# ChaissonLab/danbing-tk

Hardware: AMD Instinct MI355X
Metric: paired reads/sec aligned to RPGG (k=21) (higher is better)
Workload: dtype u64; 1 GPU; release-scale synthetic RPGG (80000 loci, 143352206 index keys, 31153328 TR k-mers) replicated per GPU; 10000000 x 150bp PE reads per GPU per step, 2% of pairs from loci; -k 21 -kf 4 1 -cth 45 -ka; RCCL all-reduce of counts at the end; lanes=1, reads_per_gpu=10000000, read_len=150, k=21, cth=45

## Files before the change

### danbing-tk_amd/csrc/dbtk_probe2.h

```cpp
#ifndef DBTK_PROBE2_H_
#define DBTK_PROBE2_H_

namespace dbtk {

#ifndef DBTK_P2_RCH
#define DBTK_P2_RCH 40
#endif
constexpr int P2_RCH = DBTK_P2_RCH;
constexpr int P2_ROW = 9;
constexpr int P2_CACHE = 128;
struct P2FuseArgs {
    uint64_t* counts; uint64_t* nmapread; uint64_t* kmc;
    uint32_t* gen_list; uint32_t* ngen; uint32_t* walk_dst;
    const uint8_t* qc;
    const ClsSlot* cls; uint64_t cls_mask; uint32_t cls_shift;
    uint64_t* pstats;
    uint64_t* ctr;
    uint32_t ctr_rep;
    dbtk_params_t P;
};
template <int NPL>
struct __attribute__((aligned(16))) Probe2SmemT {
    uint32_t pk[2][20];
    uint16_t vd[2][40];
    uint32_t rb[64 * NPL];
    union {
        uint4 stg[P2_RCH][P2_ROW];
        uint32_t res[2][2][32 * NPL];
    };
    uint4 cache[P2_CACHE];
    uint8_t tok[P2_CACHE];
    uint32_t gbuf[64];
    uint32_t fc[12];
    P2FuseArgs fa;
};
constexpr uint32_t P2_HWIN = 2048;
constexpr uint32_t P2_REP_DONE = 24, P2_REP_CLS = 25, P2_REP_INC = 26, P2_REP_SHARED = 27;
#ifndef DBTK_P2_SHARED_MAX
#define DBTK_P2_SHARED_MAX 48
#endif
constexpr uint32_t P2_SHARED_MAX = DBTK_P2_SHARED_MAX;
static_assert(P2_HWIN / 2 * 4 <= sizeof(uint4) * P2_RCH * P2_ROW, "the counter window fits where the buckets were");

template <int NPL, int WN>
DBTK_HD void sliding_min(const uint32_t (&f)[NPL + WN - 1], uint32_t (&out)[NPL]) {
    static_assert(WN >= NPL, "the windows of one lane share at least one element");
    uint32_t c = f[NPL - 1];
#pragma unroll
    for (int t = NPL; t < WN; ++t) c = f[t] < c ? f[t] : c;
    uint32_t suf[NPL];
    suf[NPL - 1] = 0xFFFFFFFFu;
#pragma unroll
    for (int j = NPL - 2; j >= 0; --j) suf[j] = f[j] < suf[j + 1] ? f[j] : suf[j + 1];
    uint32_t pre = 0xFFFFFFFFu;
#pragma unroll
    for (int j = 0; j < NPL; ++j) {
        uint32_t v = suf[j] < c ? suf[j] : c;
        out[j] = pre < v ? pre : v;
        if (j + 1 < NPL) pre = f[WN + j] < pre ? f[WN + j] : pre;
    }
}

#ifdef DBTK_STAMPS
#define P2_DIAG_MASK(a) (((a).P.diag & 512) ? 127u : 0xFFFFFFFFu)
#else
#define P2_DIAG_MASK(a) 0xFFFFFFFFu
#endif
typedef uint32_t p2_v4u __attribute__((vector_size(16)));
DBTK_HD void p2_fetch_runs(const uint32_t* rb, const MzBucket* mz, uint32_t nruns, uint32_t r0, uint32_t fq8, uint32_t part, uint32_t bmask,
                           p2_v4u (&q)[P2_RCH / 8]) {
#pragma unroll
    for (int u = 0; u < P2_RCH / 8; ++u) {
        const uint32_t run = r0 + 8 * u + fq8;
        const uint32_t b = rb[run < nruns ? run : 0u] & bmask;
        q[u] = reinterpret_cast<const p2_v4u*>(mz + (run < nruns ? (size_t)b : (size_t)0))[part];
    }
}

template <int NPL> struct P2Rv { uint64_t v[NPL]; };
enum { P2C_QC, P2C_KF, P2C_THR, P2C_FEAS, P2C_ASGN, P2C_CLS, P2C_INC, P2C_NHASH1, P2C_DONE, P2C_VV, P2C_SHARED, P2C_HF };
template <int NPL, class SM, class X>
DBTK_HD_NOINLINE void p2_resolve_gone(X& x, SM& sm_, P2Rv<NPL> rv, uint32_t nk, uint32_t gmask, uint32_t rsh, uint32_t k) {
    SM& sm = DBTK_LDS_REF(SM, sm_);
    const int lane = x.lane();
    const uint32_t hl = (uint32_t)lane & 31u, half = (uint32_t)lane >> 5, p0 = hl * NPL, cth = sm.fa.P.cthreshold;
    const bool mygone = ((gmask >> half) & 1u) != 0;
    uint32_t mc = 0;
#pragma unroll
    for (int j = 0; j < NPL; ++j) mc += (p0 + j < nk && (uint32_t)rv.v[j] == NOHIT) ? 1u : 0u;
    uint32_t ex = x.wave_excl_scan(mc);
    const uint32_t ex32 = x.bcast(ex, 32);
    if (half) ex -= ex32;
    uint32_t upto = 0;
    if (mygone && nk >= cth) {
        const uint32_t target = nk - cth + 1;
#pragma unroll
        for (int j = 0; j < NPL; ++j)
            if (p0 + j < nk && (uint32_t)rv.v[j] == NOHIT) { ++ex; if (ex == target) upto = p0 + j + 1; }
    }
    if (!mygone) upto = nk;
    upto = x.half_max(upto);
    const uint32_t looked = x.bcast(upto, 0) + x.bcast(upto, 32);
    uint32_t nvv = 0;
    if (gmask != 3u) {
        bool sh[NPL];
        bool any = false;
#pragma unroll
        for (int j = 0; j < NPL; ++j) {
            sh[j] = !mygone && p0 + j < nk && (uint32_t)rv.v[j] != NOHIT && ((uint32_t)rv.v[j] & 1u);
            any |= sh[j];
        }
        if (x.ballot(any)) {
            const uint64_t kmask = (1ull << (2 * k)) - 1;
            const uint64_t W = window_fw_clean(sm.pk[half], rsh + p0, 32), RW = revcomp2(W, 32);
            uint64_t km[NPL];
            uint32_t mine = 0, dup = 0;
#pragma unroll
            for (int j = 0; j < NPL; ++j) {
                const uint64_t fw = (W >> (2 * (32 - k - j))) & kmask, rc = (RW >> (2 * j)) & kmask;
                km[j] = fw < rc ? fw : rc;
                mine += sh[j] ? 1u : 0u;
            }
#pragma unroll
            for (int j = 0; j < NPL; ++j) {
                uint64_t mj = x.ballot(sh[j]);
                while (mj) {
                    const int src = (int)__builtin_ctzll(mj);
                    mj &= mj - 1;
                    const uint64_t ke = ((uint64_t)x.bcast((uint32_t)(km[j] >> 32), src) << 32) | x.bcast((uint32_t)km[j], src);
#pragma unroll
                    for (int j2 = j; j2 < NPL; ++j2)
                        if (sh[j2] && km[j2] == ke && (j2 > j || lane > src)) dup |= 1u << j2;
                }
            }
            nvv = x.wave_sum(mine) - x.wave_sum((uint32_t)__builtin_popcount(dup));
        }
    }
    if (lane == 0) {
        sm.fc[P2C_NHASH1] += looked;
        sm.fc[P2C_KF] += (gmask & 1u) + (gmask >> 1);
        if (gmask != 3u) { sm.fc[P2C_HF] += 1; sm.fc[P2C_VV] += nvv; }
    }
}
template <int NPL, class SM, class X>
DBTK_HD_NOINLINE void p2_resolve_usual(X& x, SM& sm_, P2Rv<NPL> rv, uint32_t nk, uint32_t v0, uint32_t nks, uint32_t t) {
    SM& sm = DBTK_LDS_REF(SM, sm_);
    const int lane = x.lane();
    const uint32_t hl = (uint32_t)lane & 31u, half = (uint32_t)lane >> 5, p0 = hl * NPL;
    const P2FuseArgs& fa = sm.fa;
    auto tally = [&](int w, uint32_t v) { if (lane == 0) sm.fc[w] += v; };
    tally(P2C_DONE, 1);
    tally(P2C_NHASH1, nks);
    const uint32_t dst = v0 >> 1;
#if defined(DBTK_STAMPS) || defined(DBTK_LF_DIAG)
    if (fa.P.diag & 64) return;
#endif
    if (fa.P.qc && fa.qc && !fa.qc[dst]) { tally(P2C_QC, 2); return; }
    if (fa.P.threading) {
        tally(P2C_THR, 2);
        if (fa.P.threading == DBTK_THREADING_V13 && lane == 0) fa.walk_dst[t] = dst;
        return;
    }
    tally(P2C_THR, 2); tally(P2C_FEAS, 2);
    if (fa.P.extract) return;
    tally(P2C_CLS, nks);
    bool kn[NPL], tr[NPL];
    uint32_t anyk = 0, anyt = 0;
#pragma unroll
    for (int j = 0; j < NPL; ++j) {
        const uint32_t ax = (uint32_t)(rv.v[j] >> 32);
        kn[j] = p0 + j < nk && (uint32_t)rv.v[j] != NOHIT && ax != CLS_NONE;
        tr[j] = kn[j] && ax != CLS_FLANK;
        anyk |= kn[j] && !tr[j] ? 1u : 0u; anyt |= tr[j] ? 1u : 0u;
    }
    const uint64_t bt = x.ballot(anyt != 0), bf = x.ballot(anyk != 0);
    const bool t0 = (uint32_t)bt != 0, t1 = (bt >> 32) != 0, f0 = (uint32_t)bf != 0, f1 = (bf >> 32) != 0;
    bool rm = true;
    uint32_t span = 0;
    if ((t0 && f0) || (t1 && f1)) assign_halves<NPL>(x, kn, tr, p0, nk, fa.P, rm, span);
    else { const bool tmate = half ? t1 : t0; rm = !tmate; span = tmate ? nk : 0u; }
    const uint32_t rm0 = x.bcast(rm ? 1u : 0u, 0), rm1 = x.bcast(rm ? 1u : 0u, 32);
    if (rm0 && rm1) return;
    tally(P2C_ASGN, 2 - rm0 - rm1);
#if defined(DBTK_STAMPS) || defined(DBTK_LF_DIAG)
    if (fa.P.diag & 128) return;
#endif
    uint32_t mn = 0xFFFFFFFFu, mx = 0;
#pragma unroll
    for (int j = 0; j < NPL; ++j) {
        const uint32_t ax = (uint32_t)(rv.v[j] >> 32);
        if (tr[j] && !rm) { mn = ax < mn ? ax : mn; mx = ax > mx ? ax : mx; }
    }
    const uint32_t hmn2 = ~x.half_max(~mn), hmx2 = x.half_max(mx);
    const uint32_t mnA = x.bcast(hmn2, 0), mnB = x.bcast(hmn2, 32), mxA = x.bcast(hmx2, 0), mxB = x.bcast(hmx2, 32);
    const uint32_t base = mnA < mnB ? mnA : mnB, top = mxA > mxB ? mxA : mxB;
    const uint32_t win = top >= base ? (top - base + 1 < P2_HWIN ? top - base + 1 : P2_HWIN) : 0u;
    uint32_t* hist = reinterpret_cast<uint32_t*>(sm.stg);
    for (uint32_t w = (uint32_t)lane; w < (win + 1) / 2; w += 64) hist[w] = 0;
    x.sync();
    uint32_t ninc = 0;
#pragma unroll
    for (int j = 0; j < NPL; ++j) {
        const bool hit = tr[j] && !rm;
        if (hit) {
            const uint32_t ax = (uint32_t)(rv.v[j] >> 32), o = ax - base;
            if (o < win) x.lds_add(&hist[o >> 1], 1u << (16 * (o & 1)));
            else x.atomic_add(&fa.counts[ax], 1ull);
        }
        ninc += (uint32_t)__builtin_popcountll(x.ballot(hit));
    }
    tally(P2C_INC, ninc);
    x.sync();
    const uint32_t span0 = x.bcast(span, 0), span1 = x.bcast(span, 32);
#if defined(DBTK_STAMPS) || defined(DBTK_LF_DIAG)
    if (!(fa.P.diag & 16))
#endif
    if (lane == 0) {
        x.atomic_add(&fa.nmapread[dst], (uint64_t)(2 - rm0 - rm1));
        x.atomic_add(&fa.kmc[dst], (uint64_t)span0 + span1);
    }
#if defined(DBTK_STAMPS) || defined(DBTK_LF_DIAG)
    if (!(fa.P.diag & 4))
#endif
    for (uint32_t i = (uint32_t)lane; i < win; i += 64) {
        const uint32_t v = (hist[i >> 1] >> (16 * (i & 1))) & 0xFFFFu;
// ... 32 lines not shown
    uint32_t dup = 0;
#pragma unroll
    for (int j = 0; j < NPL; ++j) {
        uint64_t mj = x.ballot(sh[j]);
        while (mj) {
            const int src = (int)__builtin_ctzll(mj);
            mj &= mj - 1;
            const uint64_t ke = ((uint64_t)x.bcast((uint32_t)(km[j] >> 32), src) << 32) | x.bcast((uint32_t)km[j], src);
#pragma unroll
            for (int j2 = j; j2 < NPL; ++j2)
                if (sh[j2] && km[j2] == ke && (j2 > j || lane > src)) dup |= 1u << j2;
        }
    }
    const uint32_t nvv = nshared - x.wave_sum((uint32_t)__builtin_popcount(dup));
    if (lane == 0) { sm.fc[P2C_VV] += nvv; sm.fc[P2C_SHARED] += 1; }
    p2_resolve_usual<NPL>(x, sm, rv, nk, 2u * L, nks, t);
    return true;
}

template <int NPL, int WN, bool SEL, bool FUSE, class X>
DBTK_HD void body_probe2(X& x, const BatchArgs& a) {
    typedef Probe2SmemT<NPL> SM;
    SM& sm = *x.template smem<SM>();
    const int lane = x.lane();
    const uint32_t hl = (uint32_t)lane & 31u, half = (uint32_t)lane >> 5;
    const DevTables& T = a.T;
    const uint32_t k = T.ksize, m = T.mz_m;
    const uint32_t ns = *a.nsurv;
    const uint32_t tend = ns - a.t0 < a.tcap ? ns : a.t0 + a.tcap;
    const uint32_t npc = ns > a.t0 ? tend - a.t0 : 0;
    const uint32_t npr = SEL ? *a.nsel : npc;
    if (SEL && a.pstats && x.bid() == 0 && lane == 0 && npr) x.atomic_add(&a.pstats[6], (uint64_t)npr);
    const uint32_t per = (npr + x.nblocks() - 1) / x.nblocks();
    const uint64_t lo64 = (uint64_t)x.bid() * per;
    const uint32_t first = lo64 < npr ? (uint32_t)lo64 : npr, hi = lo64 + per < npr ? (uint32_t)(lo64 + per) : npr;
    const uint32_t lmax = 32u * NPL + m - 1;
    const uint64_t kmask = (1ull << (2 * k)) - 1;
    const uint32_t mmask = (uint32_t)((1ull << (2 * m)) - 1);
    const uint32_t p0 = hl * NPL;
    if (FUSE && lane < 12) sm.fc[lane] = 0;
    if (FUSE && lane == 0) {
        sm.fa.counts = a.counts; sm.fa.nmapread = a.nmapread; sm.fa.kmc = a.kmc; sm.fa.gen_list = a.gen_list; sm.fa.ngen = a.ngen;
        sm.fa.walk_dst = a.walk_dst; sm.fa.qc = a.T.qc; sm.fa.pstats = a.pstats; sm.fa.P = a.P;
        sm.fa.ctr = counters_of(x, a); sm.fa.ctr_rep = a.ctr_rep ? 1u : 0u;
        sm.fa.cls = a.T.cls; sm.fa.cls_mask = a.T.cls_mask; sm.fa.cls_shift = a.T.cls_shift;
    }
    const P2FuseArgs& fa = sm.fa;
    uint32_t ngb = 0;
    auto flush_gen = [&]() {
        x.sync();
        uint32_t base = 0;
        if (lane == 0) base = x.atomic_add(fa.ngen, ngb);
        base = x.bcast(base, 0);
        if ((uint32_t)lane < ngb) fa.gen_list[base + lane] = sm.gbuf[lane];
        x.sync();
        ngb = 0;
    };
    for (uint32_t e = (uint32_t)lane; e < (uint32_t)P2_CACHE; e += 64) sm.cache[e] = uint4{0xFFFFFFFFu, 0x3FFFFFFFu, 0u, 0u};
    auto place_of = [&](uint32_t i) -> uint32_t {
        const uint32_t ic = i < hi ? i : (first < hi ? first : 0u);
        return SEL ? (npr ? a.sel[ic] : 0u) : ic;
    };
    uint32_t rw0 = 0, rw1 = 0;
    uint64_t o0C = 0, o1C = 0;
    uint64_t o0B = 0, o1B = 0;
    uint32_t pairA = 0;
    uint32_t plN = 0;
    auto fetch_bytes = [&](uint64_t o0, uint64_t o1) {
        uint32_t len = (uint32_t)(o1 - o0);
        if (len > lmax) len = lmax;
        const uint64_t a0 = o0 & ~3ull;
        const uint32_t nw = ((uint32_t)(o0 - a0) + len + 3) >> 2;
        rw0 = *reinterpret_cast<const uint32_t*>(a.seq + (2 * hl < nw ? a0 + 8ull * hl : 0ull));
        rw1 = *reinterpret_cast<const uint32_t*>(a.seq + (2 * hl + 1 < nw ? a0 + 8ull * hl + 4 : 0ull));
    };
    auto fetch_offsets = [&](uint32_t pair) {
        const uint64_t r = 2 * (uint64_t)pair + half;
        o0B = a.off[r]; o1B = a.off[r + 1];
    };
    if (first < hi) {
        fetch_offsets(x.uni(a.surv[a.t0 + place_of(first)]));
        o0C = o0B; o1C = o1B;
        fetch_bytes(o0C, o1C);
        if (first + 1 < hi) fetch_offsets(x.uni(a.surv[a.t0 + place_of(first + 1)]));
        pairA = a.surv[a.t0 + place_of(first + 2)];
        plN = place_of(first + 3);
    }
    DBTK_STAMP_DECL
    for (uint32_t i = first; i < hi; ++i) {
        DBTK_STAMP(43);
        const uint64_t o0 = o0C, o1 = o1C;
        uint32_t len = (uint32_t)(o1 - o0);
        if (len > lmax) { *a.errflag = DBTK_ERR_READ_TOO_LONG; len = lmax; }
        const uint64_t a0 = o0 & ~3ull;
        const uint32_t rsh = (uint32_t)(o0 - a0);
        const uint32_t d0 = rw0, d1 = rw1;
        const uint32_t place_v = place_of(i);
        {
            const bool hasB = i + 1 < hi, hasA = i + 2 < hi;
            o0C = hasB ? o0B : 0ull; o1C = hasB ? o1B : 0ull;
            fetch_bytes(o0C, o1C);
            fetch_offsets(hasA ? x.uni(pairA) : x.uni(pairA) * 0u);
            pairA = a.surv[a.t0 + plN];
            plN = place_of(i + 4);
        }
        x.sync();
        uint32_t bad = 0;
        {
            const uint32_t c0 = pack4_b2(d0, &bad), c1 = pack4_b2(d1, &bad);
            reinterpret_cast<uint16_t*>(sm.pk[half])[hl ^ 1u] = (uint16_t)(((c0 >> 8) & 0xFF00u) | ((c1 >> 16) & 0xFFu));
        }
        const uint32_t nk = len >= k ? len - k + 1 : 0, nmm = len >= m ? len - m + 1 : 0;
        const bool clean = x.ballot(bad != 0 && 8 * hl < rsh + len) == 0;
        uint64_t rv[NPL];
        if (clean) {
            x.sync();
            const uint64_t W = window_fw_clean(sm.pk[half], rsh + p0, 32);
            const uint64_t RW = revcomp2(W, 32);
            uint32_t f[NPL + WN - 1];
#pragma unroll
            for (int j = 0; j < NPL; ++j) {
                const uint32_t fwm = (uint32_t)(W >> (2 * (32 - m - j))) & mmask, rcm = (uint32_t)(RW >> (2 * j)) & mmask;
                f[j] = p0 + j < nmm ? mmer_hash2(fwm, rcm) : 0xFFFFFFFFu;
            }
#pragma unroll
            for (int t = NPL; t < NPL + WN - 1; ++t) f[t] = x.shfl_down1(f[t - NPL]);
            uint64_t km[NPL];
            bool act[NPL];
#pragma unroll
            for (int j = 0; j < NPL; ++j) {
                const uint64_t fw = (W >> (2 * (32 - k - j))) & kmask, rc = (RW >> (2 * j)) & kmask;
                km[j] = fw < rc ? fw : rc;
                act[j] = p0 + j < nk;
                rv[j] = (uint64_t)NOHIT;
            }
            DBTK_STAMP(40);
            uint32_t mz[NPL], bk[NPL];
            sliding_min<NPL, WN>(f, mz);
            uint32_t cnt = 0;
            bool st[NPL];
#pragma unroll
            for (int j = 0; j < NPL; ++j) bk[j] = act[j] ? mz_bucket(mz[j] >> 4, (uint32_t)T.mz_mask) : 0xFFFFFFFFu;
            uint32_t prev = x.shfl_up1(bk[NPL - 1]);
            if (hl == 0) prev = 0xFFFFFFFEu;
#pragma unroll
            for (int j = 0; j < NPL; ++j) {
                st[j] = act[j] && bk[j] != prev;
                cnt += st[j] ? 1u : 0u;
                prev = bk[j];
            }
            uint32_t r = x.wave_excl_scan(cnt);
            const uint32_t nruns = x.bcast(r + cnt, 63);
            uint32_t rid[NPL];
#pragma unroll
            for (int j = 0; j < NPL; ++j) {
                if (st[j]) { sm.rb[r] = bk[j]; ++r; }
                rid[j] = r - 1;
            }
            x.sync();
            DBTK_STAMP(16);
            const uint32_t fq8 = (uint32_t)lane >> 3, part = (uint32_t)lane & 7u;
            p2_v4u q[P2_RCH / 8];
            p2_fetch_runs(sm.rb, T.mz, nruns, 0u, fq8, part, P2_DIAG_MASK(a), q);
            bool pend[NPL];
#pragma unroll
            for (int j = 0; j < NPL; ++j) pend[j] = false;
            for (uint32_t r0 = 0; r0 < nruns; r0 += P2_RCH) {
                x.sync();
#pragma unroll
                for (int u = 0; u < P2_RCH / 8; ++u) *reinterpret_cast<p2_v4u*>(&sm.stg[8 * u + fq8][part]) = q[u];
                if (r0 + P2_RCH < nruns)
                    p2_fetch_runs(sm.rb, T.mz, nruns, r0 + P2_RCH, fq8, part, P2_DIAG_MASK(a), q);
                x.sync();
#pragma unroll
                for (int j = 0; j < NPL; ++j) {
                    const uint32_t row = rid[j] - r0;
                    const bool mine = act[j] && row < (uint32_t)P2_RCH;
                    if (mine) {
                        const uint4* rp = sm.stg[row];
                        int hit = -1;
                        uint32_t w7 = 0;
#pragma unroll
                        for (int g = 0; g < 4; ++g) {
                            const uint4 kk = rp[g];
                            const uint64_t k0 = ((uint64_t)kk.y << 32) | kk.x, k1 = ((uint64_t)kk.w << 32) | kk.z;
                            if (k0 == km[j]) hit = 2 * g;
                            if ((g == 3 ? (k1 & ~MZ_TURNED) : k1) == km[j]) hit = 2 * g + 1;
                            if (g == 3) w7 = kk.w;
                        }
                        const uint32_t* pl = reinterpret_cast<const uint32_t*>(rp + 4) + 2 * (hit >= 0 ? hit : 0);
                        const uint64_t pv = (uint64_t)pl[0] | ((uint64_t)pl[1] << 32);
                        if (hit >= 0) rv[j] = pv;
                        else pend[j] = (w7 >> 31) != 0;
                    }
                }
            }
            DBTK_STAMP(18);
            bool anyp = false;
#pragma unroll
            for (int j = 0; j < NPL; ++j) anyp |= pend[j];
#ifdef DBTK_STAMPS
            if (a.P.diag & 256) anyp = false;
#endif
            if (x.ballot(anyp)) {
                uint32_t oh[NPL], oi[NPL];
                bool glob[NPL];
                anyp = false;
#pragma unroll
                for (int j = 0; j < NPL; ++j) {
                    oh[j] = ovf_hash(km[j]);
                    oi[j] = oh[j] & (uint32_t)T.ovf_mask;
                    glob[j] = false;
                    if (pend[j]) {
                        const uint4 c = sm.cache[(oh[j] >> 20) & (P2_CACHE - 1)];
                        if (c.x == (uint32_t)km[j] && c.y == (uint32_t)(km[j] >> 32)) { rv[j] = ((uint64_t)c.w << 32) | c.z; pend[j] = false; }
                        else glob[j] = true;
                    }
                    anyp |= pend[j];
                }
                if (x.ballot(anyp)) {
                    uint4 q2[NPL];
                    do {
#pragma unroll
                        for (int j = 0; j < NPL; ++j) q2[j] = reinterpret_cast<const uint4*>(T.ovf)[pend[j] ? oi[j] : 0u];
                        anyp = false;
#pragma unroll
                        for (int j = 0; j < NPL; ++j) {
                            if (!pend[j]) continue;
                            const uint64_t key = ((uint64_t)q2[j].y << 32) | q2[j].x;
                            if (key == km[j]) { rv[j] = ((uint64_t)q2[j].w << 32) | q2[j].z; pend[j] = false; }
                            else if (key == MZ_EMPTY) pend[j] = false;
                            else oi[j] = (oi[j] + 1) & (uint32_t)T.ovf_mask;
                            anyp |= pend[j];
                        }
                    } while (x.ballot(anyp));
#pragma unroll
                    for (int j = 0; j < NPL; ++j) if (glob[j]) sm.tok[(oh[j] >> 20) & (P2_CACHE - 1)] = (uint8_t)lane;
                    x.sync();
#pragma unroll
                    for (int j = 0; j < NPL; ++j) {
                        const uint32_t ce = (oh[j] >> 20) & (P2_CACHE - 1);
                        if (glob[j] && sm.tok[ce] == (uint8_t)lane)
                            sm.cache[ce] = uint4{(uint32_t)km[j], (uint32_t)(km[j] >> 32), (uint32_t)rv[j], (uint32_t)(rv[j] >> 32)};
                    }
                    x.sync();
                }
            }
            DBTK_STAMP(41);
        } else {
            uint32_t vb = 0;
#pragma unroll
            for (int e = 0; e < 8; ++e) {
                const uint32_t sidx = 8 * hl + e, by = ((e < 4 ? d0 : d1) >> (8 * (e & 3))) & 0xFFu;
                const bool ok = sidx >= rsh && sidx < rsh + len && (by == 'A' || by == 'C' || by == 'G' || by == 'T');
                vb |= (ok ? 1u : 0u) << (7 - e);
            }
            reinterpret_cast<uint8_t*>(sm.vd[half])[hl ^ 1u] = (uint8_t)vb;
            x.sync();
#pragma nounroll
            for (int j = 0; j < NPL; ++j) {
                uint64_t r1 = (uint64_t)NOHIT;
                if (p0 + j < nk) {
                    const uint64_t kq = window_kmer(sm.pk[half], sm.vd[half], rsh + p0 + j, k, nullptr, nullptr);
                    if (kq != NAN64) r1 = idx_lookup64(T, kq);
                }
                sm.res[half][0][p0 + j] = (uint32_t)r1 != NOHIT ? (uint32_t)(r1 >> 32) : AUX_MISS;
                sm.res[half][1][p0 + j] = (uint32_t)r1;
            }
            x.sync();
#pragma unroll
            for (int j = 0; j < NPL; ++j) {
                const uint32_t v = sm.res[half][1][p0 + j];
                rv[j] = (uint64_t)v | ((uint64_t)sm.res[half][0][p0 + j] << 32);
            }
        }
        {
            x.sync();
            uint32_t cnt = 0, vmx = 0, vmn = 0xFFFFFFFFu;
#pragma unroll
            for (int j = 0; j < NPL; ++j) {
                const uint32_t v = p0 + j < nk ? (uint32_t)rv[j] : NOHIT;
                const bool fnd = v != NOHIT;
                cnt += fnd ? 1u : 0u;
                vmx = fnd && v > vmx ? v : vmx;
                vmn = fnd && v < vmn ? v : vmn;
                if (!FUSE) {
                    sm.res[half][0][p0 + j] = fnd ? (uint32_t)(rv[j] >> 32) : AUX_MISS;
                    sm.res[half][1][p0 + j] = v;
                }
            }
            const uint32_t nh = x.half_sum(cnt), hmx = x.half_max(vmx), hmn = ~x.half_max(~vmn);
            const bool uniform = T.consistent && nh && hmx == hmn && !(hmx & 1u);
            bool done = false;
            if (FUSE) {
                const uint32_t cth = fa.P.cthreshold;
                P2Rv<NPL> rvs;
#pragma unroll
                for (int j = 0; j < NPL; ++j) rvs.v[j] = rv[j];
                const uint32_t nk0 = x.bcast(nk, 0), nk1 = x.bcast(nk, 32), nh0 = x.bcast(nh, 0), nh1 = x.bcast(nh, 32);
                const uint32_t v0 = x.bcast(hmx, 0), v1 = x.bcast(hmx, 32);
                const bool u0 = x.bcast(uniform ? 1u : 0u, 0) != 0, u1 = x.bcast(uniform ? 1u : 0u, 32) != 0;
                const bool gone0 = nk0 < cth || nh0 < cth, gone1 = nk1 < cth || nh1 < cth;
                if (gone0 && gone1) {
                    p2_resolve_gone<NPL>(x, sm, rvs, nk, 3u, rsh, k);
                    done = true;
                } else if (clean && gone0 != gone1 && (gone0 ? nh1 : nh0) < 2 * cth) {
                    p2_resolve_gone<NPL>(x, sm, rvs, nk, gone0 ? 1u : 2u, rsh, k);
                    done = true;
                } else if (!gone0 && !gone1 && nh0 && nh1 && u0 && u1 && v0 == v1) {
                    p2_resolve_usual<NPL>(x, sm, rvs, nk, v0, nk0 + nk1, a.t0 + place_v);
                    done = true;
                } else {
                    if (clean && !gone0 && !gone1) {
                        uint32_t cu = 0, cs = 0, umx = 0, umn = 0xFFFFFFFFu;
#pragma unroll
                        for (int j = 0; j < NPL; ++j) {
                            const uint32_t v = p0 + j < nk ? (uint32_t)rv[j] : NOHIT;
                            const bool fnd = v != NOHIT, un = fnd && !(v & 1u);
                            cu += un ? 1u : 0u; cs += fnd && !un ? 1u : 0u;
                            umx = un && v > umx ? v : umx;
                            umn = un && v < umn ? v : umn;
                        }
                        const uint32_t hu = x.half_sum(cu), hs = x.half_sum(cs), hux = x.half_max(umx), hun = ~x.half_max(~umn);
                        const uint32_t u0n = x.bcast(hu, 0), u1n = x.bcast(hu, 32), ns = x.bcast(hs, 0) + x.bcast(hs, 32);
                        const uint32_t x0 = x.bcast(hux, 0), x1 = x.bcast(hux, 32), n0 = x.bcast(hun, 0), n1 = x.bcast(hun, 32);
                        const uint32_t wx = x0 > x1 ? x0 : x1, wn = n0 < n1 ? n0 : n1;
                        if (T.consistent && ns && (SEL || ns <= P2_SHARED_MAX) && u0n + u1n >= 1 && wx == wn)
                            done = p2_resolve_shared<NPL>(x, sm, rvs, nk, rsh, k, wx >> 1, ns, nk0 + nk1, a.t0 + place_v);
                    }
                    if (!done) {
                        if (lane == 0) sm.gbuf[ngb] = a.t0 + place_v;
                        if (++ngb == 64) flush_gen();
                    }
                }
            }
            if (!done) {
                if (FUSE) {
#pragma unroll
                    for (int j = 0; j < NPL; ++j) {
                        const uint32_t v = p0 + j < nk ? (uint32_t)rv[j] : NOHIT;
                        sm.res[half][0][p0 + j] = v != NOHIT ? (uint32_t)(rv[j] >> 32) : AUX_MISS;
                        sm.res[half][1][p0 + j] = v;
                    }
                }
                const uint32_t row = 2 * x.uni(place_v) + half;
                if (hl == 0) {
                    a.hithdr[row] = (uint64_t)(nh ? hmx : NOHIT) | ((uint64_t)nh << 32) | (uniform ? HDR_UNIFORM : 0ull);
// ... 200 lines not shown
```

### danbing-tk_amd/csrc/dbtk_walkfast.h

```cpp
#ifndef DBTK_WALKFAST_H_
#define DBTK_WALKFAST_H_

namespace dbtk {

struct GrMzBuildArgs {
    const GrSlot* gr;
    uint64_t nslots;
    MzBucket* mz;
    uint32_t mask, ksize, m;
};
template <class X>
DBTK_HD void body_grmz_insert(X& x, const GrMzBuildArgs& a) {
    for (uint64_t i = (uint64_t)x.bid() * x.nthreads() + x.tid(); i < a.nslots; i += (uint64_t)x.nblocks() * x.nthreads()) {
        const GrSlot s = a.gr[i];
        if (s.kmer == NAN64) continue;
        MzBucket* b = a.mz + mz_bucket(mz_of_kmer(s.kmer, a.ksize, a.m), a.mask);
        bool placed = false;
        for (int j = 0; j < 8 && !placed; ++j)
            if (x.atomic_cas(&b->key[j], MZ_EMPTY, s.kmer) == MZ_EMPTY) { b->pl[j].val = (uint32_t)(s.li >> 32); b->pl[j].aux = (uint32_t)s.li; placed = true; }
        if (!placed) x.atomic_or(&b->key[7], MZ_TURNED);
    }
}

#ifndef DBTK_WF_R
#define DBTK_WF_R 2
#endif
constexpr uint32_t WF_R = DBTK_WF_R;
DBTK_HD int walkfast_npl(uint32_t max_read_len, uint32_t k, bool grmz) {
    if (k + 4 > 32) return 0;
    const uint32_t ext = grmz ? mz_m_for_k(k) - 1 : k - 1;
    if (max_read_len <= 32 * 3 + ext && k + 2 <= 32) return 3;
    if (max_read_len <= 32 * 5 + ext) return 5;
    return 0;
}
template <int NPL>
struct __attribute__((aligned(16))) WalkFastSmemT {
    uint32_t pk[2][20];
    uint32_t rb[64 * NPL];
    uint4 stg[P2_RCH][P2_ROW];
    uint4 cache[P2_CACHE];
    uint8_t tok[P2_CACHE];
};
struct WfState {
    uint64_t c_feas = 0, c_inc = 0;
    uint32_t rbase = 0, rleft = 0;
    uint32_t txt_base = 0, txt_left = 0;
};
template <int NPL, class X>
DBTK_HD void wf_hand_over(X& x, const WalkArgs& a, WfState& S, uint32_t i, const uint32_t* gi) {
    const int lane = x.lane();
    if (!S.rleft) {
        uint32_t b = 0;
        if (lane == 0) b = x.atomic_add(a.nslow, WF_R);
        S.rbase = x.bcast(b, 0);
        S.rleft = WF_R;
    }
    const uint32_t e = S.rbase + (WF_R - S.rleft);
    --S.rleft;
    const bool info = gi && a.slow_info && e < a.info_cap && a.info_stride == 32u * NPL;
    if (lane == 0) a.slow_list[e] = i | (info ? WALK_HAS_INFO : 0u);
    if (info) {
        uint32_t* row = a.slow_info + ((size_t)e * 2 + ((uint32_t)lane >> 5)) * (32u * NPL) + ((uint32_t)lane & 31u) * NPL;
#pragma unroll
        for (int j = 0; j < NPL; ++j) row[j] = gi[j];
    }
}
template <class X>
DBTK_HD void wf_finish(X& x, const WalkArgs& a, WfState& S) {
    if ((uint32_t)x.lane() < S.rleft) a.slow_list[S.rbase + (WF_R - S.rleft) + (uint32_t)x.lane()] = WALK_NO_ENTRY;
    S.rleft = 0;
}
template <int NPL, class X>
DBTK_HD void wf_decide(X& x, const WalkArgs& a, uint32_t i, uint32_t dst, uint32_t len, uint32_t nk, uint64_t badm, const uint64_t (&fw)[NPL],
                       const uint64_t (&cn)[NPL], const uint32_t (&gi)[NPL], const bool (&act)[NPL], WfState& S, bool texting,
                       uint32_t* lcnt = nullptr, uint32_t lcap = 0) {
    const int lane = x.lane();
    const uint32_t hl = (uint32_t)lane & 31u, half = (uint32_t)lane >> 5, p0 = hl * NPL;
    const DevTables& T = a.T;
    uint64_t& c_feas = S.c_feas; uint64_t& c_inc = S.c_inc;
    uint32_t& txt_base = S.txt_base; uint32_t& txt_left = S.txt_left;
    uint32_t go[NPL];
#pragma unroll
    for (int j = 0; j < NPL; ++j) {
        const bool isf = fw[j] == cn[j];
        const uint32_t fa = gi[j] & 0x1Fu, fb = (gi[j] >> GR_OPP) & 0x1Fu;
        go[j] = isf ? fa : fb;
    }
    uint32_t pg = x.shfl_up1(go[NPL - 1]);
    uint32_t plo = x.shfl_up1((uint32_t)fw[NPL - 1]), phi = x.shfl_up1((uint32_t)(fw[NPL - 1] >> 32));
    bool fail = false;
#pragma unroll
    for (int j = 0; j < NPL; ++j) {
        const uint64_t pv = ((uint64_t)phi << 32) | plo;
        if (act[j]) {
            if (p0 + j == 0) fail |= !(go[j] & GR_HAS);
            else fail |= !((pg & GR_HAS) && ((pg >> (uint32_t)(fw[j] & 3)) & 1) && fw[j] != pv);
        }
        pg = go[j]; plo = (uint32_t)fw[j]; phi = (uint32_t)(fw[j] >> 32);
    }
    const uint64_t failm = x.ballot(fail) | badm;
    const uint64_t nkm = x.ballot(nk > 0);
    const bool clean0 = (nkm & 1) && !(failm & 0xFFFFFFFFull), clean1 = ((nkm >> 32) & 1) && !(failm >> 32);
    if ((texting ? (clean0 && clean1) : (clean0 || clean1)) && !badm) {
        c_feas += 2;
        const uint32_t tb = T.trbeg[dst];
#pragma unroll
        for (int j = 0; j < NPL; ++j) {
            const bool hit = act[j] && (gi[j] & GR_TR);
            if (hit) { const uint32_t sl = gi[j] >> GR_SLOT_SHIFT; if (sl < lcap) x.lds_add(&lcnt[sl], 1u); else x.atomic_add(&a.counts[tb + sl], 1ull); }
            c_inc += (uint64_t)__builtin_popcountll(x.ballot(hit));
        }
        if (lane == 0) {
            a.walk_dst[i] = dst;
            a.walk_ret[i] = (uint32_t)(uint8_t)(clean0 ? 1 : WALK_NOT_EVALUATED) | ((uint32_t)(uint8_t)(clean1 ? 1 : WALK_NOT_EVALUATED) << 8);
        }
        if (texting) {
            bool f[NPL];
#pragma unroll
            for (int j = 0; j < NPL; ++j) f[j] = (gi[j] & GR_TR) != 0;
            const uint64_t f0m = x.ballot(f[0]);
            const bool fnext = lane < 63 && ((f0m >> (lane + 1)) & 1);
            const uint32_t scale = half ? 4096u : 0u;
            uint32_t chg = 0;
            bool fp = x.shfl_up1(f[NPL - 1] ? 1u : 0u) != 0;
#pragma unroll
            for (int j = 0; j < NPL; ++j) {
                if (act[j] && (p0 + j == 0 || f[j] != fp)) chg = scale + p0 + j + 1;
                fp = f[j];
            }
            const uint32_t inc = x.wave_scan_max(chg);
            uint32_t before = x.shfl_up1(inc);
            if (lane == 0 || before < scale + 1) before = scale + 1;
            uint32_t rl[NPL], ol[NPL], tot = 0;
            uint32_t st = before;
            fp = x.shfl_up1(f[NPL - 1] ? 1u : 0u) != 0;
#pragma unroll
            for (int j = 0; j < NPL; ++j) {
                if (act[j] && (p0 + j == 0 || f[j] != fp)) st = scale + p0 + j + 1;
                fp = f[j];
                const bool nx = j + 1 < NPL ? f[j + 1] : fnext;
                const bool end = act[j] && (p0 + j + 1 == nk || nx != f[j]);
                rl[j] = end ? (scale + p0 + j + 1) - st + 1 : 0u;
                ol[j] = end ? (rl[j] >= 100 ? 3u : rl[j] >= 10 ? 2u : 1u) + 1u : 0u;
                tot += ol[j];
            }
            const uint32_t ex = x.wave_excl_scan(tot), la = x.half_sum(tot);
            const uint32_t la0 = x.bcast(la, 0), la1 = x.bcast(la, 32);
            const uint32_t len0 = x.bcast(len, 0), len1 = x.bcast(len, 32);
            const uint32_t lc0 = (len0 >= 100 ? 3u : len0 >= 10 ? 2u : 1u) + 1u, lc1 = (len1 >= 100 ? 3u : len1 >= 10 ? 2u : 1u) + 1u;
            const uint32_t tlen = lc1 + 1 + la1 + 1 + lc0 + 1 + la0, need = (8 + tlen + 3) & ~3u;
            if (need > txt_left) {
                uint32_t b = 0;
                if (lane == 0) b = txt_carve(x, a);
                txt_base = x.bcast(b, 0);
                txt_left = TXT_CHUNK;
            }
            if ((uint64_t)txt_base + need <= a.txt_cap) {
                uint8_t* r = a.txt + txt_base;
                if (lane == 0) {
                    reinterpret_cast<uint32_t*>(r)[0] = dst;
                    reinterpret_cast<uint32_t*>(r)[1] = tlen;
                    a.txt_idx[a.surv[i]] = txt_base;
                    uint32_t q = w_fmt_int(r, 8, (int)len1);
                    r[q] = '='; r[q + 1] = '\t';
                    r[8 + lc1 + 1 + la1] = '\t';
                    q = w_fmt_int(r, 8 + lc1 + 1 + la1 + 1, (int)len0);
                    r[q] = '='; r[q + 1] = '\t';
                }
                uint32_t o = half ? 8 + lc1 + 1 + (ex - la0) : 8 + lc1 + 1 + la1 + 1 + lc0 + 1 + ex;
#pragma unroll
                for (int j = 0; j < NPL; ++j)
                    if (ol[j]) { const uint32_t q = w_fmt_int(r, o, (int)rl[j]); r[q] = f[j] ? '=' : '.'; o += ol[j]; }
            } else if (lane == 0 && a.errflag) *a.errflag = DBTK_ERR_OVERFLOW;
            txt_base += need; txt_left -= need;
        }
    } else if (lcnt && a.pend_locus) {
        if (lane == 0) a.walk_ret[i] = WALK_PENDING;
    } else {
        uint32_t og[NPL];
#pragma unroll
        for (int j = 0; j < NPL; ++j) {
            const bool isf = fw[j] == cn[j];
            const uint32_t fa = gi[j] & 0x1Fu, fb = (gi[j] >> GR_OPP) & 0x1Fu;
            og[j] = (isf ? (fa | (fb << GR_OPP)) : (fb | (fa << GR_OPP))) | (gi[j] & ~0x3FFu);
        }
        wf_hand_over<NPL>(x, a, S, i, badm ? nullptr : og);
    }
}

template <int NPL, int WN, class X>
DBTK_HD void body_walk_fast(X& x, const WalkArgs& a) {
    typedef WalkFastSmemT<NPL> SM;
    SM& sm = *x.template smem<SM>();
    const int lane = x.lane();
    const uint32_t hl = (uint32_t)lane & 31u, half = (uint32_t)lane >> 5;
    const DevTables& T = a.T;
    const uint32_t k = T.ksize;
    uint64_t* const ctr = a.ctr_rep ? a.ctr_rep + (size_t)(x.bid() & (W_CTR_REP - 1)) * W_CTR_STRIDE : a.counters;
    const uint32_t nsurv = a.sel ? *a.nsel : *a.nsurv;
    if (a.sel && a.pstats && x.bid() == 0 && lane == 0 && nsurv) x.atomic_add(&a.pstats[13], (uint64_t)nsurv);
    const uint32_t per = (nsurv + x.nblocks() - 1) / x.nblocks();
    const uint64_t lo64 = (uint64_t)x.bid() * per;
    const uint32_t first = lo64 < nsurv ? (uint32_t)lo64 : nsurv, hi = lo64 + per < nsurv ? (uint32_t)(lo64 + per) : nsurv;
    const uint32_t lmax = 32u * NPL + (T.grmz ? mz_m_for_k(k) : k) - 1;
    const uint64_t kmask = (1ull << (2 * k)) - 1;
    const uint32_t p0 = hl * NPL;
    for (uint32_t e = (uint32_t)lane; e < (uint32_t)P2_CACHE; e += 64) sm.cache[e] = uint4{0xFFFFFFFFu, 0xFFFFFFFFu, 0u, 0xFFFFFFFFu};
    WfState S;
    const bool texting = a.txt && (a.P.aln & 3) != 0;
    auto clampi = [&](uint32_t i) { return i < hi ? i : (first < hi ? first : 0u); };
    auto place_of = [&](uint32_t i) -> uint32_t { const uint32_t ic = clampi(i); return a.sel ? (nsurv ? a.sel[ic] : 0u) : ic; };
    uint32_t rw0 = 0, rw1 = 0;
    uint64_t o0C = 0, o1C = 0, o0B = 0, o1B = 0;
    uint32_t pairA = 0, dstA = NAN32, dstB = NAN32, dstC = NAN32, plN = 0;
    auto fetch_bytes = [&](uint64_t o0, uint64_t o1) {
        uint32_t len = (uint32_t)(o1 - o0);
        if (len > lmax) len = lmax;
        const uint64_t a0 = o0 & ~3ull;
        const uint32_t nw = ((uint32_t)(o0 - a0) + len + 3) >> 2;
        rw0 = *reinterpret_cast<const uint32_t*>(a.seq + (2 * hl < nw ? a0 + 8ull * hl : 0ull));
        rw1 = *reinterpret_cast<const uint32_t*>(a.seq + (2 * hl + 1 < nw ? a0 + 8ull * hl + 4 : 0ull));
    };
    auto fetch_offsets = [&](uint32_t pair) {
        const uint64_t r = 2 * (uint64_t)pair + half;
        o0B = a.off[r]; o1B = a.off[r + 1];
    };
    if (first < hi) {
        const uint32_t q0 = place_of(first), q1 = place_of(first + 1), q2 = place_of(first + 2);
        fetch_offsets(x.uni(a.surv[q0]));
        dstC = a.walk_dst[q0];
        o0C = o0B; o1C = o1B;
        fetch_bytes(o0C, o1C);
        if (first + 1 < hi) { fetch_offsets(x.uni(a.surv[q1])); dstB = a.walk_dst[q1]; }
        pairA = a.surv[q2]; dstA = a.walk_dst[q2];
        plN = place_of(first + 3);
    }
    for (uint32_t ii = first; ii < hi; ++ii) {
        const uint64_t o0 = o0C, o1 = o1C;
        uint32_t len = (uint32_t)(o1 - o0);
        if (len > lmax) { if (a.errflag) *a.errflag = DBTK_ERR_READ_TOO_LONG; len = lmax; }
        const uint64_t a0 = o0 & ~3ull;
        const uint32_t rsh = (uint32_t)(o0 - a0);
        const uint32_t d0 = rw0, d1 = rw1;
        const uint32_t dst = x.uni(dstC);
        const uint32_t i = x.uni(place_of(ii));
        {
            const bool hasB = ii + 1 < hi, hasA = ii + 2 < hi;
            o0C = hasB ? o0B : 0ull; o1C = hasB ? o1B : 0ull;
            fetch_bytes(o0C, o1C);
            dstC = dstB; dstB = dstA;
            fetch_offsets(hasA ? x.uni(pairA) : x.uni(pairA) * 0u);
            pairA = a.surv[plN]; dstA = a.walk_dst[plN];
            plN = place_of(ii + 4);
        }
        if (dst == NAN32) continue;
        x.sync();
        uint32_t bad = 0;
        {
            const uint32_t c0 = pack4_b2(d0, &bad), c1 = pack4_b2(d1, &bad);
            reinterpret_cast<uint16_t*>(sm.pk[half])[hl ^ 1u] = (uint16_t)(((c0 >> 8) & 0xFF00u) | ((c1 >> 16) & 0xFFu));
        }
        const uint32_t nk = len >= k ? len - k + 1 : 0;
        const uint64_t badm = x.ballot(bad != 0 && 8 * hl < rsh + len);
        x.sync();
        const uint64_t W = window_fw_clean(sm.pk[half], rsh + p0, 32);
        const uint64_t RW = revcomp2(W, 32);
        uint64_t fw[NPL], cn[NPL];
        uint32_t gi[NPL];
        uint64_t at[NPL];
        bool act[NPL], open[NPL];
        uint4 q[NPL];
        auto single = [&]() {
            bool anyo = false;
#pragma unroll
            for (int j = 0; j < NPL; ++j) {
                if (open[j]) { at[j] = hash_cls(cn[j], dst, T.gr_shift); q[j] = reinterpret_cast<const uint4*>(T.gr)[at[j]]; }
                anyo |= open[j];
            }
            while (x.ballot(anyo)) {
                anyo = false;
#pragma unroll
                for (int j = 0; j < NPL; ++j) {
                    if (!open[j]) continue;
                    if (q[j].x == (uint32_t)cn[j] && q[j].y == (uint32_t)(cn[j] >> 32) && q[j].w == dst) { gi[j] = q[j].z; open[j] = false; }
                    else if ((q[j].x & q[j].y) == 0xFFFFFFFFu) open[j] = false;
                    else { at[j] = (at[j] + 1) & T.gr_mask; q[j] = reinterpret_cast<const uint4*>(T.gr)[at[j]]; }
                    anyo |= open[j];
                }
            }
        };
#pragma unroll
        for (int j = 0; j < NPL; ++j) {
            fw[j] = (W >> (2 * (32 - k - j))) & kmask;
            const uint64_t rc = (RW >> (2 * j)) & kmask;
            cn[j] = fw[j] <= rc ? fw[j] : rc;
            act[j] = p0 + j < nk;
            at[j] = 0; gi[j] = 0; open[j] = false;
            q[j] = uint4{0xFFFFFFFFu, 0xFFFFFFFFu, 0u, 0u};
        }
        if (badm) {
            wf_hand_over<NPL>(x, a, S, i, nullptr);
            continue;
        }
        if (T.grmz) {
            const uint32_t m = mz_m_for_k(k), mmask = (uint32_t)((1ull << (2 * m)) - 1), nmm = len >= m ? len - m + 1 : 0;
            uint32_t f[NPL + WN - 1], mz[NPL], bk[NPL], rid[NPL];
#pragma unroll
            for (int j = 0; j < NPL; ++j) {
                const uint32_t fwm = (uint32_t)(W >> (2 * (32 - m - j))) & mmask, rcm = (uint32_t)(RW >> (2 * j)) & mmask;
                f[j] = p0 + j < nmm ? mmer_hash2(fwm, rcm) : 0xFFFFFFFFu;
            }
#pragma unroll
            for (int t = NPL; t < NPL + WN - 1; ++t) f[t] = x.shfl_down1(f[t - NPL]);
            sliding_min<NPL, WN>(f, mz);
            uint32_t cnt = 0;
            bool st[NPL];
#pragma unroll
            for (int j = 0; j < NPL; ++j) bk[j] = act[j] ? mz_bucket(mz[j] >> 4, (uint32_t)T.grmz_mask) : 0xFFFFFFFFu;
            uint32_t prev = x.shfl_up1(bk[NPL - 1]);
            if (hl == 0) prev = 0xFFFFFFFEu;
#pragma unroll
            for (int j = 0; j < NPL; ++j) {
                st[j] = act[j] && bk[j] != prev;
                cnt += st[j] ? 1u : 0u;
                prev = bk[j];
            }
            uint32_t r = x.wave_excl_scan(cnt);
            const uint32_t nruns = x.bcast(r + cnt, 63);
            x.sync();
#pragma unroll
            for (int j = 0; j < NPL; ++j) {
                if (st[j]) { sm.rb[r] = bk[j]; ++r; }
                rid[j] = r - 1;
            }
            x.sync();
            const uint32_t fq8 = (uint32_t)lane >> 3, part = (uint32_t)lane & 7u;
            p2_v4u qq[P2_RCH / 8];
            p2_fetch_runs(sm.rb, T.grmz, nruns, 0u, fq8, part, 0xFFFFFFFFu, qq);
            for (uint32_t r0 = 0; r0 < nruns; r0 += P2_RCH) {
                x.sync();
#pragma unroll
                for (int u = 0; u < P2_RCH / 8; ++u) *reinterpret_cast<p2_v4u*>(&sm.stg[8 * u + fq8][part]) = qq[u];
                if (r0 + P2_RCH < nruns) p2_fetch_runs(sm.rb, T.grmz, nruns, r0 + P2_RCH, fq8, part, 0xFFFFFFFFu, qq);
                x.sync();
#pragma unroll
                for (int j = 0; j < NPL; ++j) {
                    const uint32_t row = rid[j] - r0;
                    if (act[j] && row < (uint32_t)P2_RCH) {
                        const uint4* rp = sm.stg[row];
                        uint32_t mm = 0, w7 = 0;
#pragma unroll
                        for (int g = 0; g < 4; ++g) {
                            const uint4 kk = rp[g];
                            const uint64_t k0 = ((uint64_t)kk.y << 32) | kk.x, k1 = ((uint64_t)kk.w << 32) | kk.z;
                            if (k0 == cn[j]) mm |= 1u << (2 * g);
                            if ((g == 3 ? (k1 & ~MZ_TURNED) : k1) == cn[j]) mm |= 1u << (2 * g + 1);
                            if (g == 3) w7 = kk.w;
                        }
                        bool found = false;
                        while (mm) {
                            const uint32_t sl = (uint32_t)__builtin_ctz(mm);
                            mm &= mm - 1;
                            const uint32_t* pl = reinterpret_cast<const uint32_t*>(rp + 4) + 2 * sl;
                            if (pl[0] == dst) { gi[j] = pl[1]; found = true; }
                        }
                        open[j] = !found && (w7 >> 31) != 0;
                    }
                }
            }
            bool anyp = false;
#pragma unroll
            for (int j = 0; j < NPL; ++j) anyp |= open[j];
            if (x.ballot(anyp)) {
                uint32_t ce[NPL];
                bool glob[NPL];
#pragma unroll
                for (int j = 0; j < NPL; ++j) {
                    ce[j] = (ovf_hash(cn[j]) >> 20) & (P2_CACHE - 1);
                    glob[j] = false;
                    if (open[j]) {
                        const uint4 c = sm.cache[ce[j]];
                        if (c.x == (uint32_t)cn[j] && c.y == (uint32_t)(cn[j] >> 32) && c.w == dst) { gi[j] = c.z; open[j] = false; }
                        else glob[j] = true;
                    }
                }
                single();
#pragma unroll
                for (int j = 0; j < NPL; ++j) if (glob[j]) sm.tok[ce[j]] = (uint8_t)lane;
                x.sync();
#pragma unroll
                for (int j = 0; j < NPL; ++j)
                    if (glob[j] && sm.tok[ce[j]] == (uint8_t)lane) sm.cache[ce[j]] = uint4{(uint32_t)cn[j], (uint32_t)(cn[j] >> 32), gi[j], dst};
                x.sync();
            }
        } else {
#pragma unroll
            for (int j = 0; j < NPL; ++j) open[j] = act[j];
            single();
        }
        wf_decide<NPL>(x, a, i, dst, len, nk, badm, fw, cn, gi, act, S, texting);
    }
    wf_finish(x, a, S);
    if (lane == 0) {
        if (S.c_feas) x.atomic_add(&ctr[DBTK_C_FEASIBLE], S.c_feas);
        if (S.c_inc) x.atomic_add(&ctr[DBTK_C_ALGO_INC], S.c_inc);
    }
}

template <int NPL, int NW>
struct __attribute__((aligned(16))) WalkFastLocWaveSmemT {
    uint32_t pk[2][20];
};
constexpr uint32_t WFL_CNT = 2048;
template <int NPL, int NW, int IMGB>
struct __attribute__((aligned(16))) WalkFastLocSmemT {
    uint4 img[IMGB / 16];
    uint32_t cnt[WFL_CNT];
    WalkFastLocWaveSmemT<NPL, NW> w[NW];
};
template <int NPL, int NW, int IMGB, class X>
DBTK_HD void body_walk_fast_locus(X& x, const WalkArgs& a, const LocRunArgs& r) {
    typedef WalkFastLocSmemT<NPL, NW, IMGB> SM;
    constexpr int IPT = ((IMGB - (int)LOC_HDR) / 16 + NW * 64 - 1) / (NW * 64);
    SM& smb = *x.template smem<SM>();
    const int lane = x.lane();
    const uint32_t wave = (uint32_t)x.tid() >> 6;
    WalkFastLocWaveSmemT<NPL, NW>& sm = smb.w[wave];
    const uint32_t* bks = reinterpret_cast<const uint32_t*>(smb.img);
    const uint32_t hl = (uint32_t)lane & 31u, half = (uint32_t)lane >> 5;
    const DevTables& T = a.T;
    const uint32_t k = T.ksize;
    uint64_t* const ctr = a.ctr_rep ? a.ctr_rep + (size_t)(x.bid() & (W_CTR_REP - 1)) * W_CTR_STRIDE : a.counters;
    const uint32_t ifirst = r.starts[x.bid()], nitems = r.starts[x.bid() + 1];
    const uint32_t lmax = 32u * NPL + k - 1;
    const uint64_t kmask = (1ull << (2 * k)) - 1;
    const uint32_t p0 = hl * NPL;
    constexpr uint32_t S = 1;
    WfState W;
    const bool texting = a.txt && (a.P.aln & 3) != 0;
    struct Cur { uint32_t it; uint32_t i, end; };
    auto desc = [&](uint32_t it) -> uint4 { return r.items[it < nitems ? it : 0u]; };
    auto seek = [&](uint32_t it) -> Cur {
        for (;;) {
            if (it >= nitems) return Cur{it, 0u, 0u};
            const uint4 d = desc(it);
            if (d.y + wave < d.z) return Cur{it, d.y + wave, d.z};
            it += S;
        }
    };
    auto next = [&](const Cur& c) -> Cur {
        if (c.it >= nitems) return c;
        if (c.i + NW < c.end) return Cur{c.it, c.i + NW, c.end};
        return seek(c.it + S);
    };
    uint32_t rw0 = 0, rw1 = 0;
    uint64_t o0C = 0, o1C = 0, o0B = 0, o1B = 0;
    uint32_t pairA = 0, dstA = NAN32, dstB = NAN32, dstC = NAN32;
    auto fetch_bytes = [&](uint64_t o0, uint64_t o1) {
        uint32_t len = (uint32_t)(o1 - o0);
        if (len > lmax) len = lmax;
        const uint64_t a0 = o0 & ~3ull;
        const uint32_t nw = ((uint32_t)(o0 - a0) + len + 3) >> 2;
        rw0 = *reinterpret_cast<const uint32_t*>(a.seq + (2 * hl < nw ? a0 + 8ull * hl : 0ull));
        rw1 = *reinterpret_cast<const uint32_t*>(a.seq + (2 * hl + 1 < nw ? a0 + 8ull * hl + 4 : 0ull));
    };
    auto fetch_offsets = [&](uint32_t pair) {
        const uint64_t rr = 2 * (uint64_t)pair + half;
        o0B = a.off[rr]; o1B = a.off[rr + 1];
    };
    auto at_of = [&](const Cur& c) { return c.it < nitems ? c.i : 0u; };
    Cur cC = seek(ifirst), cB = next(cC), cA = next(cB);
    if (cC.it < nitems) {
        fetch_offsets(x.uni(a.surv[at_of(cC)]));
        dstC = a.walk_dst[at_of(cC)];
        o0C = o0B; o1C = o1B;
        fetch_bytes(o0C, o1C);
        if (cB.it < nitems) { fetch_offsets(x.uni(a.surv[at_of(cB)])); dstB = a.walk_dst[at_of(cB)]; }
        pairA = a.surv[at_of(cA)]; dstA = a.walk_dst[at_of(cA)];
    }
    uint4 d1 = desc(ifirst), d2 = desc(ifirst + S);
    LocusDir ld1 = r.dir[x.uni(d1.x) < T.nloci ? x.uni(d1.x) : 0u];
    for (uint32_t e = (uint32_t)x.tid(); e < WFL_CNT; e += (uint32_t)x.nthreads()) smb.cnt[e] = 0;
    uint32_t trb_prev = 0;
    auto flush_counts = [&]() {
        for (uint32_t e = (uint32_t)x.tid(); e < WFL_CNT; e += (uint32_t)x.nthreads()) {
            const uint32_t v = smb.cnt[e];
            if (v) { x.atomic_add(&a.counts[trb_prev + e], (uint64_t)v); smb.cnt[e] = 0; }
        }
    };
    for (uint32_t item = ifirst; item < nitems; item += S) {
        const uint4 d = d1;
        const LocusDir ld = ld1;
        const uint32_t locus = x.uni(d.x), lgnb = x.uni(ld.lgnb), trb = x.uni(ld.trbeg);
        x.bsync();
        flush_counts();
        trb_prev = trb;
        {
            const p2_v4u* src = reinterpret_cast<const p2_v4u*>(r.arena + 16ull * ld.off16 + LOC_HDR);
            const uint32_t n16 = (ld.bytes - LOC_HDR) / 16;
            p2_v4u t[IPT];
#pragma unroll
// ... 235 lines not shown
```

Baseline: 9.479 billion reads/s.

## Stage all minimizer buckets in one pass with padded LDS rows and shared rb

Raises the per-chunk run capacity of the probe2 bucket staging from 40 to 72, so most reads fetch all their buckets in a single pass with two barriers instead of a chunked loop. The run-bucket list now lives at the tail of the staging area to save LDS, and rows are padded one slot every two rows instead of every row. A fallback chunk loop with a smaller chunk keeps long reads correct. The walkfast path keeps its own 40-run staging. This trades more live vector registers and a larger LDS footprint, which may lower occupancy. A host-only histogram of run counts is also added.

After: 9.531 billion reads/s, median of 6. Within noise of the previous version (+0.6%).

```diff
diff --git a/danbing-tk_amd/csrc/dbtk_probe2.h b/danbing-tk_amd/csrc/dbtk_probe2.h
--- a/danbing-tk_amd/csrc/dbtk_probe2.h
+++ b/danbing-tk_amd/csrc/dbtk_probe2.h
@@ -4,10 +4,27 @@
 namespace dbtk {
 
 #ifndef DBTK_P2_RCH
-#define DBTK_P2_RCH 40
+#define DBTK_P2_RCH 72
+#endif
+#ifndef DBTK_P2_PAD_EVERY
+#define DBTK_P2_PAD_EVERY 2
+#endif
+#ifndef DBTK_P2_RB_IN_STG
+#define DBTK_P2_RB_IN_STG 1
 #endif
 constexpr int P2_RCH = DBTK_P2_RCH;
-constexpr int P2_ROW = 9;
+constexpr int P2_PAD_EVERY = DBTK_P2_PAD_EVERY;
+constexpr int p2_row_g(int r) { return 8 * r + (P2_PAD_EVERY ? r / P2_PAD_EVERY : 0); }
+constexpr int P2_STG_G = p2_row_g(P2_RCH);
+static_assert(P2_RCH % 8 == 0 && P2_RCH >= 16, "whole load instructions of 8 runs");
+constexpr int p2_rch2(int npl) {
+    if (!DBTK_P2_RB_IN_STG) return P2_RCH;
+    int r = P2_RCH;
+    while (r > 0 && p2_row_g(r) * 16 + 64 * npl * 4 > P2_STG_G * 16) r -= 8;
+    return r;
+}
+constexpr int WF_RCH = 40, WF_ROW = 9;
+template <bool B> struct P2Bool { static constexpr bool value = B; };
 constexpr int P2_CACHE = 128;
 struct P2FuseArgs {
     uint64_t* counts; uint64_t* nmapread; uint64_t* kmc;
@@ -23,11 +40,20 @@
 struct __attribute__((aligned(16))) Probe2SmemT {
     uint32_t pk[2][20];
     uint16_t vd[2][40];
-    uint32_t rb[64 * NPL];
+#if !DBTK_P2_RB_IN_STG
+    uint32_t rb_own[64 * NPL];
+#endif
     union {
-        uint4 stg[P2_RCH][P2_ROW];
+        uint4 stg[P2_STG_G];
         uint32_t res[2][2][32 * NPL];
     };
+    DBTK_HD uint32_t* rb() {
+#if DBTK_P2_RB_IN_STG
+        return reinterpret_cast<uint32_t*>(&stg[0]) + (sizeof(stg) / 4 - 64 * NPL);
+#else
+        return rb_own;
+#endif
+    }
     uint4 cache[P2_CACHE];
     uint8_t tok[P2_CACHE];
     uint32_t gbuf[64];
@@ -40,7 +66,7 @@
 #define DBTK_P2_SHARED_MAX 48
 #endif
 constexpr uint32_t P2_SHARED_MAX = DBTK_P2_SHARED_MAX;
-static_assert(P2_HWIN / 2 * 4 <= sizeof(uint4) * P2_RCH * P2_ROW, "the counter window fits where the buckets were");
+static_assert(P2_HWIN / 2 * 4 <= sizeof(uint4) * P2_STG_G, "the counter window fits where the buckets were");
 
 template <int NPL, int WN>
 DBTK_HD void sliding_min(const uint32_t (&f)[NPL + WN - 1], uint32_t (&out)[NPL]) {
@@ -66,11 +92,22 @@
 #else
 #define P2_DIAG_MASK(a) 0xFFFFFFFFu
 #endif
+#if !defined(__HIPCC__)
+inline uint64_t g_p2_nruns_hist[64 * 5 + 1];
+extern "C" __attribute__((used, visibility("default"))) inline void dbtk_p2_nruns_hist(uint64_t* out, int reset) {
+    for (int i = 0; i <= 64 * 5; ++i) { if (out) out[i] = g_p2_nruns_hist[i]; if (reset) g_p2_nruns_hist[i] = 0; }
+}
+#define P2_NOTE_RUNS(lane, n) do { if ((lane) == 0) __atomic_fetch_add(&g_p2_nruns_hist[(n) <= 64 * 5 ? (n) : 64 * 5], 1ull, __ATOMIC_RELAXED); } while (0)
+#else
+#define P2_NOTE_RUNS(lane, n) do {} while (0)
+#endif
 typedef uint32_t p2_v4u __attribute__((vector_size(16)));
+template <int N, int M>
 DBTK_HD void p2_fetch_runs(const uint32_t* rb, const MzBucket* mz, uint32_t nruns, uint32_t r0, uint32_t fq8, uint32_t part, uint32_t bmask,
-                           p2_v4u (&q)[P2_RCH / 8]) {
-#pragma unroll
-    for (int u = 0; u < P2_RCH / 8; ++u) {
+                           p2_v4u (&q)[M]) {
+    static_assert(N <= M, "a register per load");
+#pragma unroll
+    for (int u = 0; u < N; ++u) {
         const uint32_t run = r0 + 8 * u + fq8;
         const uint32_t b = rb[run < nruns ? run : 0u] & bmask;
         q[u] = reinterpret_cast<const p2_v4u*>(mz + (run < nruns ? (size_t)b : (size_t)0))[part];
@@ -409,32 +446,28 @@
             uint32_t r = x.wave_excl_scan(cnt);
             const uint32_t nruns = x.bcast(r + cnt, 63);
             uint32_t rid[NPL];
+            uint32_t* const rb = sm.rb();
 #pragma unroll
             for (int j = 0; j < NPL; ++j) {
-                if (st[j]) { sm.rb[r] = bk[j]; ++r; }
+                if (st[j]) { rb[r] = bk[j]; ++r; }
                 rid[j] = r - 1;
             }
+            P2_NOTE_RUNS(lane, nruns);
             x.sync();
             DBTK_STAMP(16);
             const uint32_t fq8 = (uint32_t)lane >> 3, part = (uint32_t)lane & 7u;
             p2_v4u q[P2_RCH / 8];
-            p2_fetch_runs(sm.rb, T.mz, nruns, 0u, fq8, part, P2_DIAG_MASK(a), q);
             bool pend[NPL];
 #pragma unroll
             for (int j = 0; j < NPL; ++j) pend[j] = false;
-            for (uint32_t r0 = 0; r0 < nruns; r0 += P2_RCH) {
-                x.sync();
-#pragma unroll
-                for (int u = 0; u < P2_RCH / 8; ++u) *reinterpret_cast<p2_v4u*>(&sm.stg[8 * u + fq8][part]) = q[u];
-                if (r0 + P2_RCH < nruns)
-                    p2_fetch_runs(sm.rb, T.mz, nruns, r0 + P2_RCH, fq8, part, P2_DIAG_MASK(a), q);
-                x.sync();
+            auto search = [&](auto whole, uint32_t r0, uint32_t nrow) {
+                constexpr bool WHOLE = decltype(whole)::value;
 #pragma unroll
                 for (int j = 0; j < NPL; ++j) {
-                    const uint32_t row = rid[j] - r0;
-                    const bool mine = act[j] && row < (uint32_t)P2_RCH;
+                    const uint32_t row = WHOLE ? rid[j] : rid[j] - r0;
+                    const bool mine = WHOLE ? act[j] : act[j] && row < nrow;
                     if (mine) {
-                        const uint4* rp = sm.stg[row];
+                        const uint4* rp = sm.stg + (8 * row + (P2_PAD_EVERY ? row / (uint32_t)P2_PAD_EVERY : 0u));
                         int hit = -1;
                         uint32_t w7 = 0;
 #pragma unroll
@@ -450,6 +483,28 @@
                         if (hit >= 0) rv[j] = pv;
                         else pend[j] = (w7 >> 31) != 0;
                     }
+                }
+            };
+            if (nruns <= (uint32_t)P2_RCH) {
+                p2_fetch_runs<P2_RCH / 8>(rb, T.mz, nruns, 0u, fq8, part, P2_DIAG_MASK(a), q);
+                x.sync();
+#pragma unroll
+                for (int u = 0; u < P2_RCH / 8; ++u) *reinterpret_cast<p2_v4u*>(&sm.stg[p2_row_g(8 * u) + 8 * fq8 + (P2_PAD_EVERY ? (fq8 + (8 * u) % P2_PAD_EVERY) / (uint32_t)P2_PAD_EVERY : 0u) + part]) = q[u];
+                x.sync();
+                search(P2Bool<true>{}, 0u, 0u);
+            } else {
+                constexpr int RCH2 = p2_rch2(NPL);
+                static_assert(RCH2 >= 8 && RCH2 <= P2_RCH, "the chunk loop has rows of its own");
+                static_assert(!DBTK_P2_RB_IN_STG || p2_row_g(RCH2) * 16 + 64 * NPL * 4 <= P2_STG_G * 16, "a chunk leaves the bucket numbers alone");
+                p2_fetch_runs<RCH2 / 8>(rb, T.mz, nruns, 0u, fq8, part, P2_DIAG_MASK(a), q);
+                for (uint32_t r0 = 0; r0 < nruns; r0 += RCH2) {
+                    x.sync();
+#pragma unroll
+                    for (int u = 0; u < RCH2 / 8; ++u) *reinterpret_cast<p2_v4u*>(&sm.stg[p2_row_g(8 * u) + 8 * fq8 + (P2_PAD_EVERY ? (fq8 + (8 * u) % P2_PAD_EVERY) / (uint32_t)P2_PAD_EVERY : 0u) + part]) = q[u];
+                    if (r0 + RCH2 < nruns)
+                        p2_fetch_runs<RCH2 / 8>(rb, T.mz, nruns, r0 + RCH2, fq8, part, P2_DIAG_MASK(a), q);
+                    x.sync();
+                    search(P2Bool<false>{}, r0, (uint32_t)RCH2);
                 }
             }
             DBTK_STAMP(18);
diff --git a/danbing-tk_amd/csrc/dbtk_walkfast.h b/danbing-tk_amd/csrc/dbtk_walkfast.h
--- a/danbing-tk_amd/csrc/dbtk_walkfast.h
+++ b/danbing-tk_amd/csrc/dbtk_walkfast.h
@@ -37,7 +37,7 @@
 struct __attribute__((aligned(16))) WalkFastSmemT {
     uint32_t pk[2][20];
     uint32_t rb[64 * NPL];
-    uint4 stg[P2_RCH][P2_ROW];
+    uint4 stg[WF_RCH][WF_ROW];
     uint4 cache[P2_CACHE];
     uint8_t tok[P2_CACHE];
 };
@@ -335,18 +335,18 @@
             }
             x.sync();
             const uint32_t fq8 = (uint32_t)lane >> 3, part = (uint32_t)lane & 7u;
-            p2_v4u qq[P2_RCH / 8];
-            p2_fetch_runs(sm.rb, T.grmz, nruns, 0u, fq8, part, 0xFFFFFFFFu, qq);
-            for (uint32_t r0 = 0; r0 < nruns; r0 += P2_RCH) {
+            p2_v4u qq[WF_RCH / 8];
+            p2_fetch_runs<WF_RCH / 8>(sm.rb, T.grmz, nruns, 0u, fq8, part, 0xFFFFFFFFu, qq);
+            for (uint32_t r0 = 0; r0 < nruns; r0 += WF_RCH) {
                 x.sync();
 #pragma unroll
-                for (int u = 0; u < P2_RCH / 8; ++u) *reinterpret_cast<p2_v4u*>(&sm.stg[8 * u + fq8][part]) = qq[u];
-                if (r0 + P2_RCH < nruns) p2_fetch_runs(sm.rb, T.grmz, nruns, r0 + P2_RCH, fq8, part, 0xFFFFFFFFu, qq);
+                for (int u = 0; u < WF_RCH / 8; ++u) *reinterpret_cast<p2_v4u*>(&sm.stg[8 * u + fq8][part]) = qq[u];
+                if (r0 + WF_RCH < nruns) p2_fetch_runs<WF_RCH / 8>(sm.rb, T.grmz, nruns, r0 + WF_RCH, fq8, part, 0xFFFFFFFFu, qq);
                 x.sync();
 #pragma unroll
                 for (int j = 0; j < NPL; ++j) {
                     const uint32_t row = rid[j] - r0;
-                    if (act[j] && row < (uint32_t)P2_RCH) {
+                    if (act[j] && row < (uint32_t)WF_RCH) {
                         const uint4* rp = sm.stg[row];
                         uint32_t mm = 0, w7 = 0;
 #pragma unroll
```
